# jramapuram/BYOL

Measured on NVIDIA H100. Metric: images/sec, higher is better.
Workload: dtype bf16

## Files before the change

### byol_b200/csrc/conv_patch.cu

```cuda
#include <string.h>

#include "common.cuh"

namespace byol {

struct PatchParams {
  void* dst;
  const bf16* resid;
  float* col_sum;
  float* col_sqsum;
  Fix128* fx;
  int Nimg, H, W, C;
  int Ndim, ldc;
  int Wp, TH, HB;
  int tiles_n, num_tiles;
  int num_mt;
  int nchunks;
  int flip;
  int relu;
  uint32_t patch_bytes;
};

static constexpr int P_PATCH_SLOT = 32768;
static constexpr int P_PSTAGES = 2;
static constexpr int P_BSTAGES = 2;
static constexpr int P_THREADS = 13 * 32;
static constexpr int P_ACC_LD = acc_ld(128);

__device__ __forceinline__ void tma_load_4d(uint32_t dst_smem, const CUtensorMap* tmap, uint64_t* bar, int c0, int c1,
                                            int c2, int c3) {
  asm volatile(
      "cp.async.bulk.tensor.4d.shared::cluster.global.mbarrier::complete_tx::bytes [%0], [%1, {%3, %4, %5, %6}], [%2];"
      ::"r"(dst_smem), "l"(tmap), "r"(smem_u32(bar)), "r"(c0), "r"(c1), "r"(c2), "r"(c3)
      : "memory");
}

template <int BN, bool GROUPED = false>
__global__ void __launch_bounds__(P_THREADS, 1)
conv3x3_patch_kernel(const __grid_constant__ CUtensorMap tmapX, const __grid_constant__ CUtensorMap tmapB,
                     const PatchParams p) {
  static_assert(!GROUPED || BN == 64, "grouped mode: 64-column tiles");
  constexpr int B_STAGE = BN * 128;
  constexpr int PATCH_OFF = 0;
  constexpr int B_OFF = P_PSTAGES * 2 * P_PATCH_SLOT;
  constexpr int STAGE_OUT_OFF = B_OFF + P_BSTAGES * B_STAGE;
  constexpr int ACC_OFF = STAGE_OUT_OFF + 4 * 2048;
  constexpr int BAR_OFF = ACC_OFF + 128 * P_ACC_LD * 4;
  static_assert(2 * BN <= 128, "the accumulator tile holds two 64-column M-tiles");
  extern __shared__ __align__(1024) uint8_t smem_raw[];
  uint8_t* smem = (uint8_t*)(((uintptr_t)smem_raw + 1023) & ~(uintptr_t)1023);
  uint8_t* smemP = smem + PATCH_OFF;
  uint8_t* smemB = smem + B_OFF;
  uint8_t* stage_out = smem + STAGE_OUT_OFF;
  uint64_t* pfull = (uint64_t*)(smem + BAR_OFF);
  uint64_t* pempty = pfull + P_PSTAGES;
  uint64_t* bfull = pempty + P_PSTAGES;
  uint64_t* bempty = bfull + P_BSTAGES;
  uint64_t* tfull = bempty + P_BSTAGES;
  uint64_t* tempty = tfull + 1;
  float* accbuf = reinterpret_cast<float*>(smem + ACC_OFF);

  const int warp = threadIdx.x >> 5;
  const int lane = threadIdx.x & 31;

  if (warp == 12 && lane == 0) {
    for (int s = 0; s < P_PSTAGES; ++s) { mbar_init(&pfull[s], 1u); mbar_init(&pempty[s], 2u); }
    for (int s = 0; s < P_BSTAGES; ++s) { mbar_init(&bfull[s], 1u); mbar_init(&bempty[s], 2u); }
    mbar_init(tfull, 256u);
    mbar_init(tempty, 4u);
    fence_mbar_init();
    tma_prefetch_desc(&tmapX);
    tma_prefetch_desc(&tmapB);
  }
  __syncthreads();

  if (warp < 4) {
    const bool do_stats = p.col_sum != nullptr;
    const uint32_t stage_base = smem_u32(stage_out + warp * 2048);
    float csum[BN / 32], csq[BN / 32];
#pragma unroll
    for (int i = 0; i < BN / 32; ++i) { csum[i] = 0.f; csq[i] = 0.f; }
    int local = 0;
    int stat_n0 = -1;
    for (int tile = blockIdx.x; tile < p.num_tiles; tile += gridDim.x, ++local) {
      const int tile_n = tile % p.tiles_n;
      const int mt0 = (tile / p.tiles_n) * 2;
      const int npair = (mt0 + 1 < p.num_mt) ? 2 : 1;
      const int n0 = tile_n * BN;
      if (do_stats && stat_n0 != n0) {
        if (stat_n0 >= 0) {
#pragma unroll
          for (int i = 0; i < BN / 32; ++i) {
            if (stat_n0 + i * 32 + lane < p.Ndim) {
              fix_add(p.fx + stat_n0 + i * 32 + lane, csum[i]);
              fix_add(p.fx + p.Ndim + stat_n0 + i * 32 + lane, csq[i]);
            }
            csum[i] = 0.f; csq[i] = 0.f;
          }
        }
        stat_n0 = n0;
      }
      mbar_wait(tfull, (uint32_t)(local & 1));
      for (int jp = 0; jp < npair; ++jp) {
      const int mt = mt0 + jp;
      const int n = mt / p.HB;
      const int h0 = (mt - n * p.HB) * p.TH;
      const int ml = warp * 32 + lane;
      const int orow = ml / p.Wp;
      const int ocol = ml - orow * p.Wp;
      const bool rvalid = orow < p.TH && ocol < p.W && (h0 + orow) < p.H;
      const int64_t opix = ((int64_t)n * p.H + h0 + orow) * p.W + ocol;
      const uint32_t vmask = __ballot_sync(0xffffffffu, rvalid);
#pragma unroll
      for (int ci = 0; ci < BN / 32; ++ci) {
        const int c0 = ci * 32;
        uint32_t r[32];
        acc_load_row32(accbuf + (warp * 32 + lane) * P_ACC_LD + jp * BN + c0, r);
        if (ci == BN / 32 - 1 && jp == npair - 1) {
          __syncwarp();
          if (lane == 0) mbar_arrive(tempty);
        }
        const int nbase = n0 + c0;
        if (nbase >= p.Ndim) continue;
        float v[32];
#pragma unroll
        for (int j = 0; j < 32; ++j) v[j] = __uint_as_float(r[j]);
        if (p.resid != nullptr && rvalid) {
          const bf16* rp = p.resid + opix * p.ldc + nbase;
#pragma unroll
          for (int j = 0; j < 32; j += 8) {
            if (nbase + j < p.Ndim) {
              uint4 q = *reinterpret_cast<const uint4*>(rp + j);
              const __nv_bfloat162* h = reinterpret_cast<const __nv_bfloat162*>(&q);
#pragma unroll
              for (int e = 0; e < 4; ++e) {
                float2 f = __bfloat1622float2(h[e]);
                v[j + 2 * e] += f.x;
                v[j + 2 * e + 1] += f.y;
              }
            }
          }
        }
        if (p.relu) {
#pragma unroll
          for (int j = 0; j < 32; ++j) v[j] = fmaxf(v[j], 0.f);
        }
        uint4 q[4];
#pragma unroll
        for (int j = 0; j < 4; ++j) {
          q[j].x = pack_bf16x2(v[8 * j + 0], v[8 * j + 1]);
          q[j].y = pack_bf16x2(v[8 * j + 2], v[8 * j + 3]);
          q[j].z = pack_bf16x2(v[8 * j + 4], v[8 * j + 5]);
          q[j].w = pack_bf16x2(v[8 * j + 6], v[8 * j + 7]);
        }
        if (rvalid) {
          bf16* op = reinterpret_cast<bf16*>(p.dst) + opix * p.ldc + nbase;
#pragma unroll
          for (int j = 0; j < 4; ++j)
            if (nbase + 8 * j < p.Ndim) *reinterpret_cast<uint4*>(op + 8 * j) = q[j];
        }
        if (do_stats) {
          __syncwarp();
#pragma unroll
          for (int j = 0; j < 4; ++j) {
            const uint32_t off = (uint32_t)lane * 64u + (uint32_t)((j ^ ((lane >> 1) & 3)) << 4);
            asm volatile("st.shared.v4.b32 [%0], {%1, %2, %3, %4};" ::"r"(stage_base + off), "r"(q[j].x), "r"(q[j].y),
                         "r"(q[j].z), "r"(q[j].w)
                         : "memory");
          }
          __syncwarp();
          const uint32_t jc = (uint32_t)lane >> 3, e2 = ((uint32_t)lane & 7u) * 2u;
          uint32_t offq[4];
#pragma unroll
          for (int qq = 0; qq < 4; ++qq) offq[qq] = stage_base + ((jc ^ (uint32_t)qq) << 4) + e2;
          float s1 = 0.f, s2 = 0.f;
#pragma unroll
          for (int rr = 0; rr < 32; ++rr) {
            uint16_t hv;
            asm volatile("ld.shared.u16 %0, [%1];" : "=h"(hv) : "r"(offq[(rr >> 1) & 3] + (uint32_t)rr * 64u));
            float x = __uint_as_float((uint32_t)hv << 16);
            x = ((vmask >> rr) & 1u) ? x : 0.f;
            s1 += x;
            s2 = fmaf(x, x, s2);
          }
          csum[ci] += s1;
          csq[ci] += s2;
        }
      }
      }
    }
    if (do_stats && stat_n0 >= 0) {
#pragma unroll
      for (int i = 0; i < BN / 32; ++i) {
        if (stat_n0 + i * 32 + lane < p.Ndim) {
          fix_add(p.fx + stat_n0 + i * 32 + lane, csum[i]);
          fix_add(p.fx + p.Ndim + stat_n0 + i * 32 + lane, csq[i]);
        }
      }
    }
  } else if (warp < 12) {
    const int wg = (warp - 4) >> 2;
    const bool leader = (threadIdx.x & 127) == 0;
    float d[2][BN / 2];
    int pit = 0, bit = 0, local = 0;
    for (int tile = blockIdx.x; tile < p.num_tiles; tile += gridDim.x, ++local) {
      const int mt0 = (tile / p.tiles_n) * 2;
      const int npair = (mt0 + 1 < p.num_mt) ? 2 : 1;
      for (int cc = 0; cc < p.nchunks; ++cc, ++pit) {
        const int ps = pit % P_PSTAGES;
        mbar_wait(&pfull[ps], (uint32_t)((pit / P_PSTAGES) & 1));
        const uint32_t patch = smem_u32(smemP + ps * 2 * P_PATCH_SLOT) + (uint32_t)wg * 8192u;
        int prev_bs = -1;
        for (int tap = 0; tap < 9; ++tap, ++bit) {
          const int bs = bit % P_BSTAGES;
          mbar_wait(&bfull[bs], (uint32_t)((bit / P_BSTAGES) & 1));
          const int kh = tap / 3, kw = tap - kh * 3;
          const int shift = p.flip ? ((2 - kh) * p.Wp + (2 - kw)) : (kh * p.Wp + kw);
          const uint64_t bdesc = make_smem_desc_sw128(smem_u32(smemB + bs * B_STAGE), 16, 1024);
          wg_fence();
#pragma unroll
          for (int jp = 0; jp < 2; ++jp) {
            const uint64_t adesc =
                make_smem_desc_sw128(patch + (uint32_t)jp * P_PATCH_SLOT + (uint32_t)shift * 128u, 16, 1024);
#pragma unroll
            for (int k = 0; k < 4; ++k)
              wgmma_bf16<BN, 0, 0>(d[jp], adesc + (uint64_t)(2 * k), bdesc + (uint64_t)(2 * k),
                                   (uint32_t)((cc | tap | k) != 0));
          }
          wg_commit();
          wg_wait<1>();
          if (leader && prev_bs >= 0) mbar_arrive(&bempty[prev_bs]);
          prev_bs = bs;
        }
        wg_wait<0>();
        if (leader) {
          mbar_arrive(&bempty[prev_bs]);
          mbar_arrive(&pempty[ps]);
        }
      }
      wg_fence_acc(d[0]);
      wg_fence_acc(d[1]);
      mbar_wait(tempty, (uint32_t)((local & 1) ^ 1));
      acc_store_smem<BN>(accbuf, P_ACC_LD, wg * 64, 0, d[0]);
      if (npair == 2) acc_store_smem<BN>(accbuf, P_ACC_LD, wg * 64, BN, d[1]);
      mbar_arrive(tfull);
    }
  } else {
    if (lane == 0) {
      const int my_tiles = (p.num_tiles - (int)blockIdx.x + (int)gridDim.x - 1) / (int)gridDim.x;
      const int total = my_tiles * p.nchunks;
      auto issue_patch = [&](int g) {
        const int tile = blockIdx.x + (g / p.nchunks) * gridDim.x;
        const int cc = g % p.nchunks;
        const int mt0 = (tile / p.tiles_n) * 2;
        const int npair = (mt0 + 1 < p.num_mt) ? 2 : 1;
        const int ps = g % P_PSTAGES;
        const int c0 = GROUPED ? (tile % p.tiles_n) * BN : cc * 64;
        mbar_wait(&pempty[ps], (uint32_t)(((g / P_PSTAGES) & 1) ^ 1));
        mbar_arrive_expect_tx(&pfull[ps], p.patch_bytes * (uint32_t)npair);
        for (int jp = 0; jp < npair; ++jp) {
          const int mt = mt0 + jp;
          const int n = mt / p.HB;
          const int h0 = (mt - n * p.HB) * p.TH;
          tma_load_4d(smem_u32(smemP + (ps * 2 + jp) * P_PATCH_SLOT), &tmapX, &pfull[ps], c0, -1, h0 - 1, n);
        }
      };
      int bit = 0;
      if (total > 0) issue_patch(0);
      for (int g = 0; g < total; ++g) {
        const int tile = blockIdx.x + (g / p.nchunks) * gridDim.x;
        const int cc = g % p.nchunks;
        const int n0 = (tile % p.tiles_n) * BN;
        for (int tap = 0; tap < 9; ++tap, ++bit) {
          if (tap == 4 && g + 1 < total) issue_patch(g + 1);
          const int bs = bit % P_BSTAGES;
          mbar_wait(&bempty[bs], (uint32_t)(((bit / P_BSTAGES) & 1) ^ 1));
          mbar_arrive_expect_tx(&bfull[bs], (uint32_t)B_STAGE);
          tma_load_2d(smem_u32(smemB + bs * B_STAGE), &tmapB, &bfull[bs], (tap * p.nchunks + cc) * 64, n0);
        }
      }
    }
    __syncwarp();
  }
}

template <int BN, bool GROUPED = false>
static int launch_patch(const CUtensorMap& tx, const CUtensorMap& tb, const PatchParams& p, int sms,
                        cudaStream_t stream) {
  constexpr int SMEM = P_PSTAGES * 2 * P_PATCH_SLOT + P_BSTAGES * BN * 128 + 4 * 2048 + 128 * P_ACC_LD * 4 + 256 + 1024;
  static_assert(SMEM <= 232448, "conv3x3_patch_kernel: shared memory");
  auto kern = conv3x3_patch_kernel<BN, GROUPED>;
  if (smem_opt_in((const void*)kern, SMEM, "conv3x3_patch_kernel") != 0) return -2;
  int grid = sms < p.num_tiles ? sms : p.num_tiles;
  kern<<<grid, P_THREADS, SMEM, stream>>>(tx, tb, p);
  return check_launch("conv3x3_patch_kernel");
}

static int tmap_nhwc(CUtensorMap* tm, const void* base, int Nimg, int H, int W, int C, int box_w, int box_h,
                     const char* what) {
  const uint64_t dims[4] = {(uint64_t)C, (uint64_t)W, (uint64_t)H, (uint64_t)Nimg};
  const uint64_t strides[3] = {(uint64_t)C * 2, (uint64_t)W * C * 2, (uint64_t)H * W * C * 2};
  const uint32_t box[4] = {64u, (uint32_t)box_w, (uint32_t)box_h, 1u};
  return tmap_bf16(tm, base, 4, dims, strides, box, CU_TENSOR_MAP_SWIZZLE_128B, what);
}

bool patch_conv_applicable(int H, int W, int C, int Ndim, int KH, int KW, int stride, int pad, int out_fp32,
                           const float* bias, int64_t src_elems) {
  if (KH != 3 || KW != 3 || stride != 1 || pad != 1 || out_fp32 || bias != nullptr) return false;
  if (C % 64 != 0 || Ndim % 8 != 0) return false;
  const int Wp = W + 2;
  if (Wp > 128 || W < 12) return false;
  const int TH = 128 / Wp;
  if (128 * (128 + 2 * Wp + 2) > P_PATCH_SLOT) return false;
  if (128 * Wp * (TH + 2) > P_PATCH_SLOT) return false;
  (void)H; (void)src_elems;
  return true;
}

int patch_conv_launch(const void* src, const void* wt, void* dst, const void* resid, float* col_sum, float* col_sqsum,
                      int Nimg, int H, int W, int C, int Ndim, int ldw, int ldc, int flip, int relu, int sms,
                      cudaStream_t stream, int grouped) {
  PatchParams p;
  memset(&p, 0, sizeof(p));
  p.dst = dst; p.resid = (const bf16*)resid; p.col_sum = col_sum; p.col_sqsum = col_sqsum;
  p.Nimg = Nimg; p.H = H; p.W = W; p.C = C; p.Ndim = Ndim; p.ldc = ldc;
  p.Wp = W + 2;
  p.TH = 128 / p.Wp;
  if (p.TH > H) p.TH = H;
  p.HB = (H + p.TH - 1) / p.TH;
  const int BN = 64;
  p.tiles_n = (Ndim + BN - 1) / BN;
  p.num_mt = Nimg * p.HB;
  p.num_tiles = ((p.num_mt + 1) / 2) * p.tiles_n;
  p.nchunks = grouped ? 1 : C / 64;
  p.flip = flip;
  p.relu = relu;
  p.patch_bytes = 128u * (uint32_t)p.Wp * (uint32_t)(p.TH + 2);

  CUtensorMap tx, tb;
  if (tmap_nhwc(&tx, src, Nimg, H, W, C, p.Wp, p.TH + 2, "conv3x3_patch X") != 0) return -3;
  if (tmap_2d(&tb, wt, (uint64_t)Ndim, (uint64_t)(9 * 64 * p.nchunks), (uint64_t)ldw, (uint32_t)BN, 64u,
              "conv3x3_patch B") != 0)
    return -3;
  if (col_sum != nullptr) {
    p.fx = fix_scratch(stream, 2 * (int64_t)Ndim);
    if (p.fx == nullptr) return -2;
  }
  int rc = grouped ? launch_patch<64, true>(tx, tb, p, sms, stream) : launch_patch<64>(tx, tb, p, sms, stream);
  if (rc != 0 || col_sum == nullptr) return rc;
  return fix_flush_stats(p.fx, col_sum, col_sqsum, Ndim, stream);
}

}

namespace byol {

struct WPatchParams {
  float* dw;
  Fix128* fx;
  int Nimg, H, W, C, Cout;
  int Wp, TH, HB, num_mt;
  int co_tiles, ci_groups;
  int splits, mt_per_split;
  uint32_t patch_bytes;
  uint32_t dy_bytes;
  int gs;
};

static constexpr int WP_STAGES = 2;

static constexpr int WP_THREADS = 9 * 32;

template <int NB, bool GROUPED = false>
__global__ void __launch_bounds__(WP_THREADS, 1)
conv3x3_wgrad_patch_kernel(const __grid_constant__ CUtensorMap tmapX, const __grid_constant__ CUtensorMap tmapDY,
                           const WPatchParams p) {
  static_assert(!GROUPED || NB == 2, "grouped mode: two 64-channel patches per stage");
  constexpr int NW = GROUPED ? 64 : 64 * NB;
  constexpr int X_STAGE = NB * P_PATCH_SLOT;
  constexpr int DY_STAGE = 2 * 16384;
  constexpr int DY_OFF = WP_STAGES * X_STAGE;
  constexpr int BAR_OFF = DY_OFF + WP_STAGES * DY_STAGE;
  extern __shared__ __align__(1024) uint8_t smem_raw[];
  uint8_t* smem = (uint8_t*)(((uintptr_t)smem_raw + 1023) & ~(uintptr_t)1023);
  uint8_t* smemX = smem;
  uint8_t* smemDY = smem + DY_OFF;
  uint64_t* full_bar = (uint64_t*)(smem + BAR_OFF);
  uint64_t* empty_bar = full_bar + WP_STAGES;

  const int warp = threadIdx.x >> 5;
  const int lane = threadIdx.x & 31;
  int bid = blockIdx.x;
  const int kh = bid % 3;               bid /= 3;
  const int cig = bid % p.ci_groups;    bid /= p.ci_groups;
  const int tile_co = bid % p.co_tiles; bid /= p.co_tiles;
  const int split = bid;
  const int co0 = tile_co * 128;
  const int ci0 = GROUPED ? co0 : cig * 64 * NB;
  const int mt_begin = split * p.mt_per_split;
  int mt_end = mt_begin + p.mt_per_split;
  if (mt_end > p.num_mt) mt_end = p.num_mt;
  const int ntiles = mt_end - mt_begin;

  for (int i = threadIdx.x; i < BAR_OFF / 16; i += blockDim.x) reinterpret_cast<uint4*>(smem)[i] = make_uint4(0, 0, 0, 0);
  fence_proxy_async_smem();
  if (warp == 8 && lane == 0) {
    for (int s = 0; s < WP_STAGES; ++s) { mbar_init(&full_bar[s], 1u); mbar_init(&empty_bar[s], 2u); }
    fence_mbar_init();
    tma_prefetch_desc(&tmapX);
    tma_prefetch_desc(&tmapDY);
  }
  __syncthreads();

  if (warp == 8) {
    if (lane == 0) {
      for (int it = 0; it < ntiles; ++it) {
        const int mt = mt_begin + it;
        const int n = mt / p.HB;
        const int h0 = (mt - n * p.HB) * p.TH;
        const int s = it % WP_STAGES;
        mbar_wait(&empty_bar[s], (uint32_t)(((it / WP_STAGES) & 1) ^ 1));
        mbar_arrive_expect_tx(&full_bar[s], (uint32_t)NB * p.patch_bytes + 2u * p.dy_bytes);
#pragma unroll
        for (int c = 0; c < NB; ++c)
          tma_load_4d(smem_u32(smemX + s * X_STAGE + c * P_PATCH_SLOT), &tmapX, &full_bar[s], ci0 + 64 * c, -1, h0 - 1, n);
#pragma unroll
        for (int j = 0; j < 2; ++j)
          tma_load_4d(smem_u32(smemDY + s * DY_STAGE + j * 16384), &tmapDY, &full_bar[s], co0 + 64 * j, 0, h0, n);
      }
    }
    __syncwarp();
  } else {
    const int wg = warp >> 2;
    const bool leader = (threadIdx.x & 127) == 0;
    float d[3][NW / 2];
    int prev_s = -1;
    for (int it = 0; it < ntiles; ++it) {
      const int s = it % WP_STAGES;
      mbar_wait(&full_bar[s], (uint32_t)((it / WP_STAGES) & 1));
      const uint32_t a_base = smem_u32(smemDY + s * DY_STAGE) + (uint32_t)wg * 16384u;
      const uint32_t x_base = smem_u32(smemX + s * X_STAGE) + (GROUPED ? (uint32_t)wg * P_PATCH_SLOT : 0u);
      wg_fence();
#pragma unroll
      for (int kw = 0; kw < 3; ++kw) {
        const uint32_t shift = (uint32_t)(kh * p.Wp + kw) * 128u;
        const uint64_t adesc = make_smem_desc_sw128(a_base, 16384, 1024);
        const uint64_t bdesc = make_smem_desc_sw128(x_base + shift, P_PATCH_SLOT, 1024);
#pragma unroll
        for (int k = 0; k < 8; ++k)
          wgmma_bf16<NW, 1, 1>(d[kw], adesc + (uint64_t)(128 * k), bdesc + (uint64_t)(128 * k),
                               (uint32_t)((it | k) != 0));
      }
      wg_commit();
      wg_wait<1>();
      if (leader && prev_s >= 0) mbar_arrive(&empty_bar[prev_s]);
      prev_s = s;
    }
    wg_wait<0>();
#pragma unroll
    for (int kw = 0; kw < 3; ++kw) wg_fence_acc(d[kw]);
    const int t = threadIdx.x & 127;
    const int r0 = co0 + wg * 64 + (t >> 5) * 16 + ((t & 31) >> 2);
    if (GROUPED) {
      const int gs = p.gs;
#pragma unroll
      for (int kw = 0; kw < 3; ++kw) {
#pragma unroll
        for (int i = 0; i < NW / 2; ++i) {
          const int co = r0 + ((i & 2) ? 8 : 0);
          const int ci = ci0 + wg * 64 + 8 * (i >> 2) + 2 * (t & 3) + (i & 1);
          if (co < p.Cout && co / gs == ci / gs)
            fix_add(p.fx + ((int64_t)co * gs + ci % gs) * 9 + kh * 3 + kw, d[kw][i]);
        }
      }
      return;
    }
#pragma unroll
    for (int kw = 0; kw < 3; ++kw) {
#pragma unroll
      for (int i = 0; i < 32 * NB; ++i) {
        const int co = r0 + ((i & 2) ? 8 : 0);
        const int ci = ci0 + 8 * (i >> 2) + 2 * (t & 3) + (i & 1);
        if (co < p.Cout && ci < p.C) fix_add(p.fx + ((int64_t)co * p.C + ci) * 9 + kh * 3 + kw, d[kw][i]);
      }
    }
  }
}

template <int NB, bool GROUPED = false>
static int launch_wpatch(const CUtensorMap& tx, const CUtensorMap& ty, const WPatchParams& p, int grid,
                         cudaStream_t stream) {
  constexpr int SMEM = WP_STAGES * (NB * P_PATCH_SLOT + 2 * 16384) + 256 + 1024;
  auto kern = conv3x3_wgrad_patch_kernel<NB, GROUPED>;
  if (smem_opt_in((const void*)kern, SMEM, "conv3x3_wgrad_patch_kernel") != 0) return -2;
  kern<<<grid, WP_THREADS, SMEM, stream>>>(tx, ty, p);
  return check_launch("conv3x3_wgrad_patch_kernel");
}

bool patch_wgrad_applicable(int H, int W, int C, int Cin_real, int Cout, int KH, int KW, int stride, int pad) {
  if (KH != 3 || KW != 3 || stride != 1 || pad != 1) return false;
  if (C % 64 != 0 || C != Cin_real || Cout % 8 != 0) return false;
  const int Wp = W + 2;
  if (Wp > 128 || W < 12) return false;
  if (128 * (128 + 2 * Wp + 2) > P_PATCH_SLOT) return false;
  (void)H;
  return true;
}

int patch_wgrad_launch(const void* x, const void* dy, float* dw, int Nimg, int H, int W, int C, int Cout, int sms,
                       cudaStream_t stream, int gs) {
  WPatchParams p;
  memset(&p, 0, sizeof(p));
  p.dw = dw; p.Nimg = Nimg; p.H = H; p.W = W; p.C = C; p.Cout = Cout;
  p.Wp = W + 2;
  p.TH = 128 / p.Wp;
  if (p.TH > H) p.TH = H;
  p.HB = (H + p.TH - 1) / p.TH;
  p.num_mt = Nimg * p.HB;
  constexpr int NB = 1;
  p.gs = gs;
  p.co_tiles = (Cout + 127) / 128;
  p.ci_groups = gs > 0 ? 1 : C / (64 * NB);
  const int base = p.co_tiles * p.ci_groups * 3;
  int splits = sms / base;
  if (splits < 1) splits = 1;
  if (splits > p.num_mt) splits = p.num_mt;
  p.mt_per_split = (p.num_mt + splits - 1) / splits;
  p.splits = (p.num_mt + p.mt_per_split - 1) / p.mt_per_split;
  p.patch_bytes = 128u * (uint32_t)p.Wp * (uint32_t)(p.TH + 2);
  p.dy_bytes = 128u * (uint32_t)p.Wp * (uint32_t)p.TH;
  CUtensorMap tx, ty;
  if (tmap_nhwc(&tx, x, Nimg, H, W, C, p.Wp, p.TH + 2, "conv3x3_wgrad_patch X") != 0) return -3;
  if (tmap_nhwc(&ty, dy, Nimg, H, W, Cout, p.Wp, p.TH, "conv3x3_wgrad_patch dY") != 0) return -3;
  const int grid = base * p.splits;
  const int64_t ndw = (int64_t)Cout * (gs > 0 ? gs : C) * 9;
  p.fx = fix_scratch(stream, ndw);
  if (p.fx == nullptr) return -2;
  const int rc = gs > 0 ? launch_wpatch<2, true>(tx, ty, p, grid, stream) : launch_wpatch<NB>(tx, ty, p, grid, stream);
  return fix_done(stream, rc != 0 ? rc : fix_flush(p.fx, dw, ndw, stream));
}

}
```

Before: 2340.

## Add bf16 accumulator hand-off path with 128-column tiles and deferred stats replay

For convolutions without residual or relu, the MMA warps now write bf16-packed swizzled accumulators straight to shared memory, replacing the fp32 buffer. The epilogue copies them out directly. When Ndim exceeds 64 the kernel uses 128-column tiles with one M-tile and eight B stages, which gives more reuse of each patch load. Column statistics for that mode are written as per-M-tile partials and reduced by a separate replay kernel, then the partials are cleared with a memset. This adds an extra kernel, partial-buffer traffic and a memset, and it rounds values to bf16 before computing the stats.

```diff
diff --git a/byol_b200/csrc/conv_patch.cu b/byol_b200/csrc/conv_patch.cu
--- a/byol_b200/csrc/conv_patch.cu
+++ b/byol_b200/csrc/conv_patch.cu
@@ -10,6 +10,7 @@
   float* col_sum;
   float* col_sqsum;
   Fix128* fx;
+  float* part;
   int Nimg, H, W, C;
   int Ndim, ldc;
   int Wp, TH, HB;
@@ -23,9 +24,25 @@
 
 static constexpr int P_PATCH_SLOT = 32768;
 static constexpr int P_PSTAGES = 2;
-static constexpr int P_BSTAGES = 2;
 static constexpr int P_THREADS = 13 * 32;
-static constexpr int P_ACC_LD = acc_ld(128);
+
+template <int BN, bool H16>
+struct PatchLayout {
+  static constexpr int MT = (H16 && BN == 128) ? 1 : 2;
+  static constexpr int BSTAGES = H16 ? 8 : 2;
+  static constexpr int B_STAGE = BN * 128;
+  static constexpr int ACC_LD = acc_ld(128);
+  static constexpr int MT_BYTES = 128 * BN * 2;
+  static constexpr int PATCH_OFF = 0;
+  static constexpr int B_OFF = P_PSTAGES * MT * P_PATCH_SLOT;
+  static constexpr int STAGE_OUT_OFF = B_OFF + BSTAGES * B_STAGE;
+  static constexpr int ACC_OFF = STAGE_OUT_OFF + (H16 ? 0 : 4 * 2048);
+  static constexpr int BAR_OFF = ACC_OFF + (H16 ? MT * MT_BYTES : 128 * ACC_LD * 4);
+  static constexpr int SMEM = BAR_OFF + 256 + 1024;
+  static_assert(H16 || 2 * BN <= 128, "the fp32 accumulator tile holds two 64-column M-tiles");
+  static_assert(BN == 64 || (H16 && BN == 128), "patch tiles: 64 columns, or 128 with the bf16 hand-off");
+  static_assert(SMEM <= 232448, "conv3x3_patch_kernel: one CTA per SM, <= 227 KB of dynamic shared memory");
+};
 
 __device__ __forceinline__ void tma_load_4d(uint32_t dst_smem, const CUtensorMap* tmap, uint64_t* bar, int c0, int c1,
                                             int c2, int c3) {
@@ -35,37 +52,34 @@
       : "memory");
 }
 
-template <int BN, bool GROUPED = false>
+template <int BN, bool GROUPED = false, bool H16 = false>
 __global__ void __launch_bounds__(P_THREADS, 1)
 conv3x3_patch_kernel(const __grid_constant__ CUtensorMap tmapX, const __grid_constant__ CUtensorMap tmapB,
                      const PatchParams p) {
-  static_assert(!GROUPED || BN == 64, "grouped mode: 64-column tiles");
-  constexpr int B_STAGE = BN * 128;
-  constexpr int PATCH_OFF = 0;
-  constexpr int B_OFF = P_PSTAGES * 2 * P_PATCH_SLOT;
-  constexpr int STAGE_OUT_OFF = B_OFF + P_BSTAGES * B_STAGE;
-  constexpr int ACC_OFF = STAGE_OUT_OFF + 4 * 2048;
-  constexpr int BAR_OFF = ACC_OFF + 128 * P_ACC_LD * 4;
-  static_assert(2 * BN <= 128, "the accumulator tile holds two 64-column M-tiles");
+  static_assert(!GROUPED || (BN == 64 && !H16), "grouped mode: 64-column tiles, fp32 hand-off");
+  using L = PatchLayout<BN, H16>;
+  constexpr int MT = L::MT;
+  constexpr int BST = L::BSTAGES;
   extern __shared__ __align__(1024) uint8_t smem_raw[];
   uint8_t* smem = (uint8_t*)(((uintptr_t)smem_raw + 1023) & ~(uintptr_t)1023);
-  uint8_t* smemP = smem + PATCH_OFF;
-  uint8_t* smemB = smem + B_OFF;
-  uint8_t* stage_out = smem + STAGE_OUT_OFF;
-  uint64_t* pfull = (uint64_t*)(smem + BAR_OFF);
+  uint8_t* smemP = smem + L::PATCH_OFF;
+  uint8_t* smemB = smem + L::B_OFF;
+  uint8_t* stage_out = smem + L::STAGE_OUT_OFF;
+  uint64_t* pfull = (uint64_t*)(smem + L::BAR_OFF);
   uint64_t* pempty = pfull + P_PSTAGES;
   uint64_t* bfull = pempty + P_PSTAGES;
-  uint64_t* bempty = bfull + P_BSTAGES;
-  uint64_t* tfull = bempty + P_BSTAGES;
+  uint64_t* bempty = bfull + BST;
+  uint64_t* tfull = bempty + BST;
   uint64_t* tempty = tfull + 1;
-  float* accbuf = reinterpret_cast<float*>(smem + ACC_OFF);
+  float* accbuf = reinterpret_cast<float*>(smem + L::ACC_OFF);
+  const uint32_t tile16 = smem_u32(smem + L::ACC_OFF);
 
   const int warp = threadIdx.x >> 5;
   const int lane = threadIdx.x & 31;
 
   if (warp == 12 && lane == 0) {
     for (int s = 0; s < P_PSTAGES; ++s) { mbar_init(&pfull[s], 1u); mbar_init(&pempty[s], 2u); }
-    for (int s = 0; s < P_BSTAGES; ++s) { mbar_init(&bfull[s], 1u); mbar_init(&bempty[s], 2u); }
+    for (int s = 0; s < BST; ++s) { mbar_init(&bfull[s], 1u); mbar_init(&bempty[s], 2u); }
     mbar_init(tfull, 256u);
     mbar_init(tempty, 4u);
     fence_mbar_init();
@@ -76,18 +90,35 @@
 
   if (warp < 4) {
     const bool do_stats = p.col_sum != nullptr;
+    const bool reg_stats = do_stats && MT == 2;
     const uint32_t stage_base = smem_u32(stage_out + warp * 2048);
     float csum[BN / 32], csq[BN / 32];
 #pragma unroll
     for (int i = 0; i < BN / 32; ++i) { csum[i] = 0.f; csq[i] = 0.f; }
     int local = 0;
     int stat_n0 = -1;
+    auto block_sums = [&](uint32_t blk, uint32_t vmask, float& s1, float& s2) {
+      const uint32_t jc = (uint32_t)lane >> 3, e2 = ((uint32_t)lane & 7u) * 2u;
+      uint32_t offq[4];
+#pragma unroll
+      for (int qq = 0; qq < 4; ++qq) offq[qq] = blk + ((jc ^ (uint32_t)qq) << 4) + e2;
+      s1 = 0.f; s2 = 0.f;
+#pragma unroll
+      for (int rr = 0; rr < 32; ++rr) {
+        uint16_t hv;
+        asm volatile("ld.shared.u16 %0, [%1];" : "=h"(hv) : "r"(offq[(rr >> 1) & 3] + (uint32_t)rr * 64u));
+        float x = __uint_as_float((uint32_t)hv << 16);
+        x = ((vmask >> rr) & 1u) ? x : 0.f;
+        s1 += x;
+        s2 = fmaf(x, x, s2);
+      }
+    };
     for (int tile = blockIdx.x; tile < p.num_tiles; tile += gridDim.x, ++local) {
       const int tile_n = tile % p.tiles_n;
-      const int mt0 = (tile / p.tiles_n) * 2;
-      const int npair = (mt0 + 1 < p.num_mt) ? 2 : 1;
+      const int mt0 = (tile / p.tiles_n) * MT;
+      const int npair = (MT == 2 && mt0 + 1 < p.num_mt) ? 2 : 1;
       const int n0 = tile_n * BN;
-      if (do_stats && stat_n0 != n0) {
+      if (reg_stats && stat_n0 != n0) {
         if (stat_n0 >= 0) {
 #pragma unroll
           for (int i = 0; i < BN / 32; ++i) {
@@ -111,11 +142,49 @@
       const bool rvalid = orow < p.TH && ocol < p.W && (h0 + orow) < p.H;
       const int64_t opix = ((int64_t)n * p.H + h0 + orow) * p.W + ocol;
       const uint32_t vmask = __ballot_sync(0xffffffffu, rvalid);
+      if constexpr (H16) {
+        const uint32_t qbase = tile16 + (uint32_t)jp * L::MT_BYTES + (uint32_t)warp * (BN / 32) * 2048u;
+#pragma unroll
+        for (int ci = 0; ci < BN / 32; ++ci) {
+          const int nbase = n0 + ci * 32;
+          if (nbase >= p.Ndim) continue;
+          const uint32_t blk = qbase + (uint32_t)ci * 2048u;
+          if (rvalid) {
+            bf16* op = reinterpret_cast<bf16*>(p.dst) + opix * p.ldc + nbase;
+#pragma unroll
+            for (int j = 0; j < 4; ++j) {
+              uint4 q;
+              asm volatile("ld.shared.v4.b32 {%0, %1, %2, %3}, [%4];"
+                           : "=r"(q.x), "=r"(q.y), "=r"(q.z), "=r"(q.w)
+                           : "r"(blk + (uint32_t)lane * 64u + (uint32_t)((j ^ ((lane >> 1) & 3)) << 4)));
+              if (nbase + 8 * j < p.Ndim) *reinterpret_cast<uint4*>(op + 8 * j) = q;
+            }
+          }
+          if (do_stats) {
+            float s1, s2;
+            block_sums(blk, vmask, s1, s2);
+            if (MT == 1) {
+              const int64_t o = ((int64_t)mt * 4 + warp) * p.Ndim + nbase + lane;
+              if (nbase + lane < p.Ndim) {
+                p.part[o] = s1;
+                p.part[(int64_t)p.num_mt * 4 * p.Ndim + o] = s2;
+              }
+            } else {
+              csum[ci] += s1;
+              csq[ci] += s2;
+            }
+          }
+        }
+        if (jp == npair - 1) {
+          __syncwarp();
+          if (lane == 0) mbar_arrive(tempty);
+        }
+      } else {
 #pragma unroll
       for (int ci = 0; ci < BN / 32; ++ci) {
         const int c0 = ci * 32;
         uint32_t r[32];
-        acc_load_row32(accbuf + (warp * 32 + lane) * P_ACC_LD + jp * BN + c0, r);
+        acc_load_row32(accbuf + (warp * 32 + lane) * L::ACC_LD + jp * BN + c0, r);
         if (ci == BN / 32 - 1 && jp == npair - 1) {
           __syncwarp();
           if (lane == 0) mbar_arrive(tempty);
@@ -169,27 +238,16 @@
                          : "memory");
           }
           __syncwarp();
-          const uint32_t jc = (uint32_t)lane >> 3, e2 = ((uint32_t)lane & 7u) * 2u;
-          uint32_t offq[4];
-#pragma unroll
-          for (int qq = 0; qq < 4; ++qq) offq[qq] = stage_base + ((jc ^ (uint32_t)qq) << 4) + e2;
-          float s1 = 0.f, s2 = 0.f;
-#pragma unroll
-          for (int rr = 0; rr < 32; ++rr) {
-            uint16_t hv;
-            asm volatile("ld.shared.u16 %0, [%1];" : "=h"(hv) : "r"(offq[(rr >> 1) & 3] + (uint32_t)rr * 64u));
-            float x = __uint_as_float((uint32_t)hv << 16);
-            x = ((vmask >> rr) & 1u) ? x : 0.f;
-            s1 += x;
-            s2 = fmaf(x, x, s2);
-          }
+          float s1, s2;
+          block_sums(stage_base, vmask, s1, s2);
           csum[ci] += s1;
           csq[ci] += s2;
         }
       }
       }
-    }
-    if (do_stats && stat_n0 >= 0) {
+      }
+    }
+    if (reg_stats && stat_n0 >= 0) {
 #pragma unroll
       for (int i = 0; i < BN / 32; ++i) {
         if (stat_n0 + i * 32 + lane < p.Ndim) {
@@ -201,25 +259,25 @@
   } else if (warp < 12) {
     const int wg = (warp - 4) >> 2;
     const bool leader = (threadIdx.x & 127) == 0;
-    float d[2][BN / 2];
+    float d[MT][BN / 2];
     int pit = 0, bit = 0, local = 0;
     for (int tile = blockIdx.x; tile < p.num_tiles; tile += gridDim.x, ++local) {
-      const int mt0 = (tile / p.tiles_n) * 2;
-      const int npair = (mt0 + 1 < p.num_mt) ? 2 : 1;
+      const int mt0 = (tile / p.tiles_n) * MT;
+      const int npair = (MT == 2 && mt0 + 1 < p.num_mt) ? 2 : 1;
       for (int cc = 0; cc < p.nchunks; ++cc, ++pit) {
         const int ps = pit % P_PSTAGES;
         mbar_wait(&pfull[ps], (uint32_t)((pit / P_PSTAGES) & 1));
-        const uint32_t patch = smem_u32(smemP + ps * 2 * P_PATCH_SLOT) + (uint32_t)wg * 8192u;
+        const uint32_t patch = smem_u32(smemP + ps * MT * P_PATCH_SLOT) + (uint32_t)wg * 8192u;
         int prev_bs = -1;
         for (int tap = 0; tap < 9; ++tap, ++bit) {
-          const int bs = bit % P_BSTAGES;
-          mbar_wait(&bfull[bs], (uint32_t)((bit / P_BSTAGES) & 1));
+          const int bs = bit % BST;
+          mbar_wait(&bfull[bs], (uint32_t)((bit / BST) & 1));
           const int kh = tap / 3, kw = tap - kh * 3;
           const int shift = p.flip ? ((2 - kh) * p.Wp + (2 - kw)) : (kh * p.Wp + kw);
-          const uint64_t bdesc = make_smem_desc_sw128(smem_u32(smemB + bs * B_STAGE), 16, 1024);
+          const uint64_t bdesc = make_smem_desc_sw128(smem_u32(smemB + bs * L::B_STAGE), 16, 1024);
           wg_fence();
 #pragma unroll
-          for (int jp = 0; jp < 2; ++jp) {
+          for (int jp = 0; jp < MT; ++jp) {
             const uint64_t adesc =
                 make_smem_desc_sw128(patch + (uint32_t)jp * P_PATCH_SLOT + (uint32_t)shift * 128u, 16, 1024);
 #pragma unroll
@@ -238,11 +296,17 @@
           mbar_arrive(&pempty[ps]);
         }
       }
-      wg_fence_acc(d[0]);
-      wg_fence_acc(d[1]);
+#pragma unroll
+      for (int jp = 0; jp < MT; ++jp) wg_fence_acc(d[jp]);
       mbar_wait(tempty, (uint32_t)((local & 1) ^ 1));
-      acc_store_smem<BN>(accbuf, P_ACC_LD, wg * 64, 0, d[0]);
-      if (npair == 2) acc_store_smem<BN>(accbuf, P_ACC_LD, wg * 64, BN, d[1]);
+      if constexpr (H16) {
+        const uint32_t wbase = tile16 + (uint32_t)wg * 2u * (BN / 32) * 2048u;
+        acc_store_bf16_sw64<BN>(wbase, d[0]);
+        if (MT == 2 && npair == 2) acc_store_bf16_sw64<BN>(wbase + (uint32_t)L::MT_BYTES, d[MT - 1]);
+      } else {
+        acc_store_smem<BN>(accbuf, L::ACC_LD, wg * 64, 0, d[0]);
+        if (npair == 2) acc_store_smem<BN>(accbuf, L::ACC_LD, wg * 64, BN, d[MT - 1]);
+      }
       mbar_arrive(tfull);
     }
   } else {
@@ -252,8 +316,8 @@
       auto issue_patch = [&](int g) {
         const int tile = blockIdx.x + (g / p.nchunks) * gridDim.x;
         const int cc = g % p.nchunks;
-        const int mt0 = (tile / p.tiles_n) * 2;
-        const int npair = (mt0 + 1 < p.num_mt) ? 2 : 1;
+        const int mt0 = (tile / p.tiles_n) * MT;
+        const int npair = (MT == 2 && mt0 + 1 < p.num_mt) ? 2 : 1;
         const int ps = g % P_PSTAGES;
         const int c0 = GROUPED ? (tile % p.tiles_n) * BN : cc * 64;
         mbar_wait(&pempty[ps], (uint32_t)(((g / P_PSTAGES) & 1) ^ 1));
@@ -262,7 +326,7 @@
           const int mt = mt0 + jp;
           const int n = mt / p.HB;
           const int h0 = (mt - n * p.HB) * p.TH;
-          tma_load_4d(smem_u32(smemP + (ps * 2 + jp) * P_PATCH_SLOT), &tmapX, &pfull[ps], c0, -1, h0 - 1, n);
+          tma_load_4d(smem_u32(smemP + (ps * MT + jp) * P_PATCH_SLOT), &tmapX, &pfull[ps], c0, -1, h0 - 1, n);
         }
       };
       int bit = 0;
@@ -273,10 +337,10 @@
         const int n0 = (tile % p.tiles_n) * BN;
         for (int tap = 0; tap < 9; ++tap, ++bit) {
           if (tap == 4 && g + 1 < total) issue_patch(g + 1);
-          const int bs = bit % P_BSTAGES;
-          mbar_wait(&bempty[bs], (uint32_t)(((bit / P_BSTAGES) & 1) ^ 1));
-          mbar_arrive_expect_tx(&bfull[bs], (uint32_t)B_STAGE);
-          tma_load_2d(smem_u32(smemB + bs * B_STAGE), &tmapB, &bfull[bs], (tap * p.nchunks + cc) * 64, n0);
+          const int bs = bit % BST;
+          mbar_wait(&bempty[bs], (uint32_t)(((bit / BST) & 1) ^ 1));
+          mbar_arrive_expect_tx(&bfull[bs], (uint32_t)L::B_STAGE);
+          tma_load_2d(smem_u32(smemB + bs * L::B_STAGE), &tmapB, &bfull[bs], (tap * p.nchunks + cc) * 64, n0);
         }
       }
     }
@@ -284,16 +348,62 @@
   }
 }
 
-template <int BN, bool GROUPED = false>
+template <int BN, bool GROUPED = false, bool H16 = false>
 static int launch_patch(const CUtensorMap& tx, const CUtensorMap& tb, const PatchParams& p, int sms,
                         cudaStream_t stream) {
-  constexpr int SMEM = P_PSTAGES * 2 * P_PATCH_SLOT + P_BSTAGES * BN * 128 + 4 * 2048 + 128 * P_ACC_LD * 4 + 256 + 1024;
-  static_assert(SMEM <= 232448, "conv3x3_patch_kernel: shared memory");
-  auto kern = conv3x3_patch_kernel<BN, GROUPED>;
+  constexpr int SMEM = PatchLayout<BN, H16>::SMEM;
+  auto kern = conv3x3_patch_kernel<BN, GROUPED, H16>;
   if (smem_opt_in((const void*)kern, SMEM, "conv3x3_patch_kernel") != 0) return -2;
   int grid = sms < p.num_tiles ? sms : p.num_tiles;
   kern<<<grid, P_THREADS, SMEM, stream>>>(tx, tb, p);
   return check_launch("conv3x3_patch_kernel");
+}
+
+__global__ void __launch_bounds__(256) patch_stats_replay_kernel(const float* __restrict__ part, Fix128* __restrict__ fx,
+                                                                 int Ndim, int num_mt, int tiles_n, int num_tiles) {
+  constexpr int U = 8;
+  const int quarter = threadIdx.x >> 6, j = threadIdx.x & 63;
+  const int64_t plane = (int64_t)num_mt * 4 * Ndim;
+  float csum = 0.f, csq = 0.f;
+  int stat_col = -1;
+  for (int tile0 = blockIdx.x; tile0 < num_tiles; tile0 += U * gridDim.x) {
+    float v[U][4];
+#pragma unroll
+    for (int u = 0; u < U; ++u) {
+      const int tile = tile0 + u * gridDim.x;
+      const int col = (tile % tiles_n) * 64 + j;
+      const int mt0 = (tile / tiles_n) * 2;
+      const bool ok = tile < num_tiles && col < Ndim;
+      const bool two = ok && mt0 + 1 < num_mt;
+      const float* q0 = part + ((int64_t)mt0 * 4 + quarter) * Ndim + col;
+      v[u][0] = ok ? q0[0] : 0.f;
+      v[u][1] = ok ? q0[plane] : 0.f;
+      v[u][2] = two ? q0[4 * (int64_t)Ndim] : 0.f;
+      v[u][3] = two ? q0[plane + 4 * (int64_t)Ndim] : 0.f;
+    }
+#pragma unroll
+    for (int u = 0; u < U; ++u) {
+      const int tile = tile0 + u * gridDim.x;
+      if (tile >= num_tiles) break;
+      const int col = (tile % tiles_n) * 64 + j;
+      const int mt0 = (tile / tiles_n) * 2;
+      if (col != stat_col) {
+        if (stat_col >= 0 && stat_col < Ndim) {
+          fix_add(fx + stat_col, csum);
+          fix_add(fx + Ndim + stat_col, csq);
+        }
+        csum = 0.f; csq = 0.f;
+        stat_col = col;
+      }
+      if (col >= Ndim) continue;
+      csum += v[u][0]; csq += v[u][1];
+      if (mt0 + 1 < num_mt) { csum += v[u][2]; csq += v[u][3]; }
+    }
+  }
+  if (stat_col >= 0 && stat_col < Ndim) {
+    fix_add(fx + stat_col, csum);
+    fix_add(fx + Ndim + stat_col, csq);
+  }
 }
 
 static int tmap_nhwc(CUtensorMap* tm, const void* base, int Nimg, int H, int W, int C, int box_w, int box_h,
@@ -328,10 +438,12 @@
   p.TH = 128 / p.Wp;
   if (p.TH > H) p.TH = H;
   p.HB = (H + p.TH - 1) / p.TH;
-  const int BN = 64;
+  const bool h16 = !grouped && resid == nullptr && !relu;
+  const int BN = (h16 && Ndim > 64) ? 128 : 64;
+  const int mt_per_tile = BN == 128 ? 1 : 2;
   p.tiles_n = (Ndim + BN - 1) / BN;
   p.num_mt = Nimg * p.HB;
-  p.num_tiles = ((p.num_mt + 1) / 2) * p.tiles_n;
+  p.num_tiles = ((p.num_mt + mt_per_tile - 1) / mt_per_tile) * p.tiles_n;
   p.nchunks = grouped ? 1 : C / 64;
   p.flip = flip;
   p.relu = relu;
@@ -342,11 +454,28 @@
   if (tmap_2d(&tb, wt, (uint64_t)Ndim, (uint64_t)(9 * 64 * p.nchunks), (uint64_t)ldw, (uint32_t)BN, 64u,
               "conv3x3_patch B") != 0)
     return -3;
+  const int pair_tiles = ((p.num_mt + 1) / 2) * ((Ndim + 63) / 64);
+  const bool replay = BN == 128 && col_sum != nullptr;
   if (col_sum != nullptr) {
-    p.fx = fix_scratch(stream, 2 * (int64_t)Ndim);
+    const int64_t part_floats = replay ? 2 * (int64_t)p.num_mt * 4 * Ndim : 0;
+    p.fx = fix_scratch(stream, 2 * (int64_t)Ndim + (part_floats + 5) / 6);
     if (p.fx == nullptr) return -2;
-  }
-  int rc = grouped ? launch_patch<64, true>(tx, tb, p, sms, stream) : launch_patch<64>(tx, tb, p, sms, stream);
+    if (replay) p.part = reinterpret_cast<float*>(p.fx + 2 * (int64_t)Ndim);
+  }
+  int rc;
+  if (grouped) rc = launch_patch<64, true>(tx, tb, p, sms, stream);
+  else if (!h16) rc = launch_patch<64>(tx, tb, p, sms, stream);
+  else if (BN == 128) rc = launch_patch<128, false, true>(tx, tb, p, sms, stream);
+  else rc = launch_patch<64, false, true>(tx, tb, p, sms, stream);
+  if (rc == 0 && replay) {
+    patch_stats_replay_kernel<<<sms < pair_tiles ? sms : pair_tiles, 256, 0, stream>>>(p.part, p.fx, Ndim, p.num_mt,
+                                                                                       (Ndim + 63) / 64, pair_tiles);
+    rc = check_launch("patch_stats_replay_kernel");
+    if (rc == 0 && cudaMemsetAsync(p.part, 0, (size_t)2 * p.num_mt * 4 * Ndim * sizeof(float), stream) != cudaSuccess) {
+      set_last_error("conv3x3_patch: memset failed");
+      rc = -2;
+    }
+  }
   if (rc != 0 || col_sum == nullptr) return rc;
   return fix_flush_stats(p.fx, col_sum, col_sqsum, Ndim, stream);
 }
```

After: 2417, median of 6. +3.3%, better.
